# Jamy-L/Handheld-Multi-Frame-Super-Resolution

Measured on AMD Instinct MI355X. Metric: output Mpix/s for 12MP x 20-frame x2 SR burst; max-abs diff vs reference, higher is better.
Workload: dtype f32

## Files before the change

handheld-multi-frame-super-resolution_amd/csrc/hhsr_robustness.hip:

```cpp
#include "hhsr_common.h"

__device__ __forceinline__ double dodgson(double x) {
    const double a = fabs(x);
    if (a <= 0.5) return -2.0 * a * a + 1.0;
    if (a <= 1.5) return a * a - 5.0 / 2.0 * a + 1.5;
    return 0.0;
}

template <int NC>
__device__ __forceinline__ bool dodgson_sample(const float* __restrict__ LR, int lh, int lw, int y, int x, double fx,
                                               double fy, float out[NC]) {
    const double ly = ((double)y + fy + 0.5) / 2.0 - 0.5;
    const double lx = ((double)x + fx + 0.5) / 2.0 - 0.5;
    if (!(ly >= 0.0 && ly < (double)lh && lx >= 0.0 && lx < (double)lw)) return false;
    const int cy = (int)rint(ly), cx = (int)rint(lx);
    const size_t plane = (size_t)lh * lw;
    float b[NC];
#pragma unroll
    for (int c = 0; c < NC; ++c) b[c] = 0.f;
    double wacc = 0.0;
#pragma unroll
    for (int i = -1; i <= 1; ++i) {
        const int y_ = clampi(cy + i, 0, lh - 1);
        const double wy = dodgson((double)y_ - ly);
// ... 268 lines not shown
    w[1] = inner;
    w[2] = c + 1 <= len - 1 ? op : inner;
}

__global__ void __launch_bounds__(256) k_rob_frame_tile(const float* __restrict__ cm, int lh, int lw,
                                                         const float* __restrict__ rmean,
                                                         const float* __restrict__ ssq,
                                                         const uint32_t* __restrict__ cidx,
                                                         const float2* __restrict__ flow, int nx, int ts,
                                                         const float* __restrict__ S,
                                                         const double* __restrict__ difc, double t,
                                                         float* __restrict__ R, int H, int W) {
    __shared__ float s_g[2][2][3][RF_WN][RF_WN + 2];
    const int lx_ = threadIdx.x & (RF_BX - 1), ly_ = threadIdx.x >> 5;
    const int grp = lx_ >> 4;
    const int bx = blockIdx.x * RF_BX + grp * RF_T, by = blockIdx.y * RF_BY;
    const int x = blockIdx.x * RF_BX + lx_;
    const int tix = min(bx, W - 1) / ts;
    RobAxis ay[2], ax[2];
    int wy0[2], wx0[2];
    float Sv[2];
#pragma unroll
    for (int v = 0; v < 2; ++v) {
        const int tiy = min(by + RF_T * v, H - 1) / ts;
        const float2 f = flow[(size_t)tiy * nx + tix];
        Sv[v] = S[(size_t)tiy * nx + tix];
        ay[v] = rob_axis(f.y);
        ax[v] = rob_axis(f.x);
        float r_;
        rob_centre(ay[v], by + RF_T * v, lh, wy0[v], r_);
        rob_centre(ax[v], bx, lw, wx0[v], r_);
        wy0[v] = clampi(wy0[v], -4, lh + 4) - 1;
        wx0[v] = clampi(wx0[v], -4, lw + 4) - 1;
    }
    const size_t gplane = (size_t)lh * lw;
    const int tg = (lx_ & (RF_T - 1)) + RF_T * ly_;
    constexpr int WSZ = 3 * RF_WN * RF_WN, NST = (WSZ + 127) / 128;
    float st[2][NST];
#pragma unroll
    for (int v = 0; v < 2; ++v)
#pragma unroll
        for (int u = 0; u < NST; ++u) {
            const int p = tg + 128 * u;
            if (p < WSZ) {
                const int c = p / (RF_WN * RF_WN), q = p - c * (RF_WN * RF_WN);
                const int i = q / RF_WN, j = q - i * RF_WN;
                const int gy = clampi(wy0[v] + i, 0, lh - 1), gx = clampi(wx0[v] + j, 0, lw - 1);
                st[v][u] = cm[c * gplane + (size_t)gy * lw + gx];
            }
        }
    const size_t plane = (size_t)H * W;
    bool live[RF_NK];
    size_t o[RF_NK];
    float rb[RF_NK][3], s_sq[RF_NK];
    uint32_t ci[RF_NK];
#pragma unroll
    for (int k = 0; k < RF_NK; ++k) {
        const int y = by + ly_ + 8 * k;
        live[k] = x < W && y < H;
        o[k] = live[k] ? (size_t)y * W + x : 0;
#pragma unroll
        for (int c = 0; c < 3; ++c) rb[k][c] = rmean[c * plane + o[k]];
        s_sq[k] = ssq[o[k]];
        ci[k] = cidx[o[k]];
    }
#pragma unroll
    for (int v = 0; v < 2; ++v)
#pragma unroll
        for (int u = 0; u < NST; ++u) {
            const int p = tg + 128 * u;
            if (p < WSZ) {
                const int c = p / (RF_WN * RF_WN), q = p - c * (RF_WN * RF_WN);
                const int i = q / RF_WN, j = q - i * RF_WN;
                s_g[grp][v][c][i][j] = st[v][u];
            }
        }
    __syncthreads();
#pragma unroll
    for (int k = 0; k < RF_NK; ++k) {
        if (!live[k]) continue;
        const int v = k >> 1, y = by + ly_ + 8 * k;
        float d_t[3];
#pragma unroll
        for (int c = 0; c < 3; ++c) d_t[c] = (float)difc[(ci[k] >> (10 * c)) & 1023u];
        int cy, cx;
        float ry, rx;
        const bool iny = rob_centre(ay[v], y, lh, cy, ry), inx = rob_centre(ax[v], x, lw, cx, rx);
        float cmu[3] = {INFINITY, INFINITY, INFINITY};
        if (iny && inx) {
            float wxv[3], wyv[3], b0 = 0.f, b1 = 0.f, b2 = 0.f, wacc = 0.f;
            dodgson3(rx, cx, lw, wxv);
            dodgson3(ry, cy, lh, wyv);
            const int wi0 = cy - 1 - wy0[v], wj0 = cx - 1 - wx0[v];
#pragma unroll
            for (int i = 0; i < 3; ++i) {
#pragma unroll
                for (int j = 0; j < 3; ++j) {
                    const float w = wyv[i] * wxv[j];
                    b0 = fmaf(s_g[grp][v][0][wi0 + i][wj0 + j], w, b0);
                    b1 = fmaf(s_g[grp][v][1][wi0 + i][wj0 + j], w, b1);
                    b2 = fmaf(s_g[grp][v][2][wi0 + i][wj0 + j], w, b2);
                    wacc += w;
                }
            }
            const float iw = __builtin_amdgcn_rcpf(wacc);
            cmu[0] = b0 * iw;
            cmu[1] = b1 * iw;
            cmu[2] = b2 * iw;
        }
        float d_sq = 0.f;
#pragma unroll
        for (int c = 0; c < 3; ++c) {
            const float dp = fabsf(rb[k][c] - cmu[c]);
            const float dp2 = dp * dp;
            const float shrink = dp2 * __builtin_amdgcn_rcpf(dp2 + d_t[c] * d_t[c]);
            d_sq += dp2 * shrink * shrink;
        }
        const float e = __builtin_amdgcn_exp2f((-d_sq * __builtin_amdgcn_rcpf(s_sq[k])) * 1.44269504088896341f);
        double r = (double)(Sv[v] * e) - t;
        r = r > 0.0 ? r : 0.0;
        r = r < 1.0 ? r : 1.0;
        R[o[k]] = (float)r;
    }
}

__device__ __forceinline__ void rob_row4(const float (*win)[RF_WN][RF_WN + 2], const RobAxis& ay, const RobAxis& ax,
                                         int wy0, int wx0, int y, int x0, int lh, int lw, const float rbk[4][3],
                                         const float d_t2[4][3], const float iss[4], float Sv, float tf, float out[4]) {
    int cy;
    float ry, wyv[3];
    const bool iny = rob_centre(ay, y, lh, cy, ry);
    dodgson3(ry, cy, lh, wyv);
    const int wi0 = cy - 1 - wy0;
    float cmu[4][3];
#pragma unroll
    for (int ph = 0; ph < 2; ++ph) {
        int cx;
        float rx;
        const bool inx = rob_centre(ax, x0 + ph, lw, cx, rx);
#pragma unroll
        for (int c = 0; c < 3; ++c) cmu[ph][c] = cmu[ph + 2][c] = INFINITY;
        if (iny && inx && cx >= 1 && cx + 2 <= lw - 1) {
            float wxv[3], w[3][3], wacc = 0.f;
            dodgson3(rx, cx, lw, wxv);
#pragma unroll
            for (int i = 0; i < 3; ++i)
#pragma unroll
                for (int j = 0; j < 3; ++j) {
                    w[i][j] = wyv[i] * wxv[j];
                    wacc += w[i][j];
                }
            const float iw = __builtin_amdgcn_rcpf(wacc);
            const int wj0 = cx - 1 - wx0;
#pragma unroll
            for (int c = 0; c < 3; ++c) {
                float g4[3][4];
#pragma unroll
                for (int i = 0; i < 3; ++i)
#pragma unroll
                    for (int j = 0; j < 4; ++j) g4[i][j] = win[c][wi0 + i][wj0 + j];
#pragma unroll
                for (int q = 0; q < 2; ++q) {
                    float b = 0.f;
#pragma unroll
                    for (int i = 0; i < 3; ++i)
#pragma unroll
                        for (int j = 0; j < 3; ++j) b = fmaf(g4[i][j + q], w[i][j], b);
                    cmu[ph + 2 * q][c] = b * iw;
                }
            }
        } else {
            int cx2;
            float rx2;
            const bool inx2 = rob_centre(ax, x0 + ph + 2, lw, cx2, rx2);
#pragma unroll
            for (int q = 0; q < 2; ++q) {
                const int cxq = q ? cx2 : cx;
                const float rxq = q ? rx2 : rx;
                if (iny && (q ? inx2 : inx)) {
                    float wxv[3], b0 = 0.f, b1 = 0.f, b2 = 0.f, wacc = 0.f;
                    dodgson3(rxq, cxq, lw, wxv);
                    const int wj0 = cxq - 1 - wx0;
#pragma unroll
                    for (int i = 0; i < 3; ++i) {
#pragma unroll
                        for (int j = 0; j < 3; ++j) {
                            const float w = wyv[i] * wxv[j];
                            b0 = fmaf(win[0][wi0 + i][wj0 + j], w, b0);
                            b1 = fmaf(win[1][wi0 + i][wj0 + j], w, b1);
                            b2 = fmaf(win[2][wi0 + i][wj0 + j], w, b2);
                            wacc += w;
                        }
                    }
                    const float iw = __builtin_amdgcn_rcpf(wacc);
                    cmu[ph + 2 * q][0] = b0 * iw;
                    cmu[ph + 2 * q][1] = b1 * iw;
                    cmu[ph + 2 * q][2] = b2 * iw;
                }
            }
        }
    }
#pragma unroll
    for (int k = 0; k < 4; ++k) {
        float d_sq = 0.f;
#pragma unroll
        for (int c = 0; c < 3; ++c) {
            const float dp = fabsf(rbk[k][c] - cmu[k][c]);
            const float dp2 = dp * dp;
            const float shrink = dp2 * __builtin_amdgcn_rcpf(dp2 + d_t2[k][c]);
            d_sq += dp2 * shrink * shrink;
        }
        const float e = __builtin_amdgcn_exp2f((-d_sq * iss[k]) * 1.44269504088896341f);
        out[k] = __builtin_amdgcn_fmed3f(Sv * e - tf, 0.f, 1.f);
    }
}

__global__ void __launch_bounds__(256) k_rob_frame_row4(const float* __restrict__ cm, int lh, int lw,
                                                         const float* __restrict__ rmean,
                                                         const float* __restrict__ ssq,
                                                         const uint32_t* __restrict__ cidx,
                                                         const float2* __restrict__ flow, int nx, int ts,
                                                         const float* __restrict__ S,
                                                         const double* __restrict__ difc, double t,
                                                         float* __restrict__ R, int H, int W) {
    __shared__ float s_g[2][2][3][RF_WN][RF_WN + 2];
    const int lx4 = threadIdx.x & 7, ly_ = threadIdx.x >> 3;
    const int grp = lx4 >> 2, v = ly_ >> 4;
    const int bid = xcd_remap(blockIdx.y * gridDim.x + blockIdx.x, gridDim.x * gridDim.y);
    const int bxi = bid % gridDim.x, byi = bid / gridDim.x;
    const int sx0 = bxi * RF_BX + grp * RF_T, sy0 = byi * RF_BY + v * RF_T;
    const int x0 = bxi * RF_BX + 4 * lx4, y = byi * RF_BY + ly_;
    const int tix = min(sx0, W - 1) / ts, tiy = min(sy0, H - 1) / ts;
    const float2 f = flow[(size_t)tiy * nx + tix];
    const float Sv = S[(size_t)tiy * nx + tix];
    const RobAxis ay = rob_axis(f.y), ax = rob_axis(f.x);
    int wy0, wx0;
    {
        float r_;
        rob_centre(ay, sy0, lh, wy0, r_);
        rob_centre(ax, sx0, lw, wx0, r_);
        wy0 = clampi(wy0, -4, lh + 4) - 1;
        wx0 = clampi(wx0, -4, lw + 4) - 1;
    }
    const size_t gplane = (size_t)lh * lw;
    const int tg = (ly_ & (RF_T - 1)) * 4 + (lx4 & 3);
    constexpr int WSZ = 3 * RF_WN * RF_WN, NST = (WSZ + 63) / 64;
    float st[NST];
#pragma unroll
    for (int u = 0; u < NST; ++u) {
        const int p = tg + 64 * u;
        if (p < WSZ) {
            const int c = p / (RF_WN * RF_WN), q = p - c * (RF_WN * RF_WN);
            const int i = q / RF_WN, j = q - i * RF_WN;
            const int gy = clampi(wy0 + i, 0, lh - 1), gx = clampi(wx0 + j, 0, lw - 1);
            st[u] = cm[c * gplane + (size_t)gy * lw + gx];
        }
    }
    const size_t plane = (size_t)H * W;
    const bool live = x0 < W && y < H;
    const size_t o = live ? (size_t)y * W + x0 : 0;
    float4 rb4[3];
#pragma unroll
    for (int c = 0; c < 3; ++c) rb4[c] = *reinterpret_cast<const float4*>(rmean + c * plane + o);
    const float4 ss4 = *reinterpret_cast<const float4*>(ssq + o);
    const uint4 ci4 = *reinterpret_cast<const uint4*>(cidx + o);
#pragma unroll
    for (int u = 0; u < NST; ++u) {
        const int p = tg + 64 * u;
        if (p < WSZ) {
            const int c = p / (RF_WN * RF_WN), q = p - c * (RF_WN * RF_WN);
            const int i = q / RF_WN, j = q - i * RF_WN;
            s_g[grp][v][c][i][j] = st[u];
        }
    }
    __syncthreads();
    if (!live) return;
    const float rbk[4][3] = {{rb4[0].x, rb4[1].x, rb4[2].x}, {rb4[0].y, rb4[1].y, rb4[2].y},
                             {rb4[0].z, rb4[1].z, rb4[2].z}, {rb4[0].w, rb4[1].w, rb4[2].w}};
    const float ssk[4] = {ss4.x, ss4.y, ss4.z, ss4.w};
    const uint32_t cik[4] = {ci4.x, ci4.y, ci4.z, ci4.w};
    float d_t2[4][3], iss[4], out[4];
#pragma unroll
    for (int k = 0; k < 4; ++k) {
#pragma unroll
        for (int c = 0; c < 3; ++c) {
            const float d = (float)difc[(cik[k] >> (10 * c)) & 1023u];
            d_t2[k][c] = d * d;
        }
        iss[k] = __builtin_amdgcn_rcpf(ssk[k]);
    }
    rob_row4(s_g[grp][v], ay, ax, wy0, wx0, y, x0, lh, lw, rbk, d_t2, iss, Sv, (float)t, out);
    *reinterpret_cast<float4*>(R + o) = make_float4(out[0], out[1], out[2], out[3]);
}

constexpr int ROB_GROUP = 4;
struct RobGroup {
    const float* cm[ROB_GROUP];
    const float2* flow[ROB_GROUP];
    const float* S[ROB_GROUP];
    float* R[ROB_GROUP];
    int n;
};

__global__ void __launch_bounds__(256) k_rob_frames_row4(RobGroup gq, int lh, int lw, const float* __restrict__ rmean,
                                                          const float* __restrict__ ssq,
                                                          const uint32_t* __restrict__ cidx, int ny, int nx, int ts,
                                                          const double* __restrict__ difc, double t, int H, int W,
                                                          double Mt2, float s1, float s2, int rows_lo, int rows_hi) {
    __shared__ float s_g[2][2][3][RF_WN][RF_WN + 2];
    __shared__ float4 s_tab[ROB_GROUP][2][2][2];
    const int lx4 = threadIdx.x & 7, ly_ = threadIdx.x >> 3;
    const int grp = lx4 >> 2, v = ly_ >> 4;
    const int bid = xcd_remap(blockIdx.y * gridDim.x + blockIdx.x, gridDim.x * gridDim.y);
    const int bxi = bid % gridDim.x, byi = bid / gridDim.x;
    const int x0 = bxi * RF_BX + 4 * lx4, y = byi * RF_BY + ly_;
    const size_t gplane = (size_t)lh * lw, plane = (size_t)H * W;
    const int tg = (ly_ & (RF_T - 1)) * 4 + (lx4 & 3);
    constexpr int WSZ = 3 * RF_WN * RF_WN, NST = (WSZ + 63) / 64;
    const bool live = x0 < W && y < H;
    const size_t o = live ? (size_t)y * W + x0 : 0;
    float4 rb4[3];
#pragma unroll
    for (int c = 0; c < 3; ++c) rb4[c] = *reinterpret_cast<const float4*>(rmean + c * plane + o);
    const float4 ss4 = *reinterpret_cast<const float4*>(ssq + o);
    const uint4 ci4 = *reinterpret_cast<const uint4*>(cidx + o);
    const float rbk[4][3] = {{rb4[0].x, rb4[1].x, rb4[2].x}, {rb4[0].y, rb4[1].y, rb4[2].y},
                             {rb4[0].z, rb4[1].z, rb4[2].z}, {rb4[0].w, rb4[1].w, rb4[2].w}};
    const float ssk[4] = {ss4.x, ss4.y, ss4.z, ss4.w};
    const uint32_t cik[4] = {ci4.x, ci4.y, ci4.z, ci4.w};
    float d_t2[4][3], iss[4];
#pragma unroll
    for (int k = 0; k < 4; ++k) {
#pragma unroll
        for (int c = 0; c < 3; ++c) {
            const float d = (float)difc[(cik[k] >> (10 * c)) & 1023u];
            d_t2[k][c] = d * d;
        }
        iss[k] = __builtin_amdgcn_rcpf(ssk[k]);
    }
    if (threadIdx.x < gq.n * 4) {
        const int fr = threadIdx.x >> 2, vv = (threadIdx.x >> 1) & 1, gg = threadIdx.x & 1;
        const int tsx0 = bxi * RF_BX + gg * RF_T, tsy0 = byi * RF_BY + vv * RF_T;
        const size_t tl = (size_t)(min(tsy0, H - 1) / ts) * nx + min(tsx0, W - 1) / ts;
        const float2 f = gq.flow[fr][tl];
        const RobAxis ay = rob_axis(f.y), ax = rob_axis(f.x);
        int wy0, wx0;
        float r_;
        rob_centre(ay, tsy0, lh, wy0, r_);
        rob_centre(ax, tsx0, lw, wx0, r_);
        wy0 = clampi(wy0, -4, lh + 4) - 1;
        wx0 = clampi(wx0, -4, lw + 4) - 1;
        const int flags = (ay.lt ? 1 : 0) | (ay.eq ? 2 : 0) | (ay.ok ? 4 : 0) | (ax.lt ? 8 : 0) | (ax.eq ? 16 : 0) | (ax.ok ? 32 : 0);
        s_tab[fr][vv][gg][0] = make_float4(__int_as_float(ay.fi), ay.h, __int_as_float(wy0), __int_as_float(flags));
        float Sv;
        if (gq.S[fr]) {
            Sv = gq.S[fr][tl];
        } else {
            const int tiy = (int)(tl / nx), tix = (int)(tl - (size_t)tiy * nx);
            float mnx = INFINITY, mny = INFINITY, mxx = -INFINITY, mxy = -INFINITY;
            for (int i = -1; i <= 1; ++i)
                for (int j = -1; j <= 1; ++j) {
                    const int yy = tiy + i, xx = tix + j;
                    if (yy >= -rows_lo && yy < ny + rows_hi && xx >= 0 && xx < nx) {
                        const float2 q = gq.flow[fr][(ptrdiff_t)yy * nx + xx];
                        mxx = fmaxf(mxx, q.x); mxy = fmaxf(mxy, q.y);
                        mnx = fminf(mnx, q.x); mny = fminf(mny, q.y);
                    }
                }
            const float d0 = mxx - mnx, d1 = mxy - mny;
            const float m = d0 * d0 + d1 * d1;
            Sv = ((double)m > Mt2) ? s1 : s2;
        }
        s_tab[fr][vv][gg][1] = make_float4(__int_as_float(ax.fi), ax.h, __int_as_float(wx0), Sv);
    }
    __syncthreads();
    float st[NST];
    int fci[NST];
    unsigned fco[NST];
#pragma unroll
    for (int u = 0; u < NST; ++u) {
        const int p = tg + 64 * u;
        const int c = p / (RF_WN * RF_WN), q = p - c * (RF_WN * RF_WN);
        const int i = q / RF_WN, j = q - i * RF_WN;
        fci[u] = (i << 8) | j;
        fco[u] = (unsigned)c * (unsigned)gplane;
    }
    auto fetch = [&](int fr) {
        const float* __restrict__ cm = gq.cm[fr];
        const int wy0 = __float_as_int(s_tab[fr][v][grp][0].z), wx0 = __float_as_int(s_tab[fr][v][grp][1].z);
#pragma unroll
        for (int u = 0; u < NST; ++u) {
            const int p = tg + 64 * u;
            if (p < WSZ) {
                const int gy = clampi(wy0 + (fci[u] >> 8), 0, lh - 1), gx = clampi(wx0 + (fci[u] & 255), 0, lw - 1);
                const unsigned off = (fco[u] + (unsigned)(__mul24(gy, lw) + gx)) * 4u;
                st[u] = *reinterpret_cast<const float*>(reinterpret_cast<const char*>(cm) + off);
            }
        }
    };
    if (gq.n > 0) fetch(0);
    for (int fr = 0; fr < gq.n; ++fr) {
        const float4 t0 = s_tab[fr][v][grp][0], t1 = s_tab[fr][v][grp][1];
        const int flags = __float_as_int(t0.w);
        RobAxis ay, ax;
        ay.fi = __float_as_int(t0.x); ay.h = t0.y; ay.lt = flags & 1; ay.eq = flags & 2; ay.ok = flags & 4;
        ax.fi = __float_as_int(t1.x); ax.h = t1.y; ax.lt = flags & 8; ax.eq = flags & 16; ax.ok = flags & 32;
        const int wy0 = __float_as_int(t0.z), wx0 = __float_as_int(t1.z);
        const float Sv = t1.w;
        if (fr) __syncthreads();
#pragma unroll
        for (int u = 0; u < NST; ++u) {
            const int p = tg + 64 * u;
            if (p < WSZ) {
                const int c = p / (RF_WN * RF_WN), q = p - c * (RF_WN * RF_WN);
                const int i = q / RF_WN, j = q - i * RF_WN;
                s_g[grp][v][c][i][j] = st[u];
            }
        }
        __syncthreads();
        if (fr + 1 < gq.n) fetch(fr + 1);
        if (!live) continue;
        float out[4];
        rob_row4(s_g[grp][v], ay, ax, wy0, wx0, y, x0, lh, lw, rbk, d_t2, iss, Sv, (float)t, out);
        *reinterpret_cast<float4*>(gq.R[fr] + o) = make_float4(out[0], out[1], out[2], out[3]);
    }
}

extern "C" int hhsr_rob_frame(const float* comp_means, int lh, int lw, const float* ref_means,
                              const float* ref_sigma_sq, const uint32_t* ref_curve_index, const float* flow, int ny,
                              int nx, int ts, const float* S, const double* diff_curve, int ncurve, double t, float* R,
                              void* stream) {
    HHSR_ARG(comp_means && ref_means && ref_sigma_sq && flow && S && diff_curve && R);
    HHSR_ARG(lh > 0 && lw > 0 && ts > 0 && ncurve > 0);
    const int H = 2 * lh, W = 2 * lw;
    HHSR_ARG(ny * ts >= H && nx * ts >= W);
    const bool vec4 = W % 4 == 0 && (((uintptr_t)ref_means | (uintptr_t)ref_sigma_sq | (uintptr_t)ref_curve_index |
                                      (uintptr_t)R) & 15) == 0;
    if (ts % RF_T == 0 && ref_curve_index && ncurve <= 1024 && vec4)
        hipLaunchKernelGGL(k_rob_frame_row4, dim3(hhsr_cdiv(W, RF_BX), hhsr_cdiv(H, RF_BY)), dim3(256), 0,
                           (hipStream_t)stream, comp_means, lh, lw, ref_means, ref_sigma_sq, ref_curve_index,
                           reinterpret_cast<const float2*>(flow), nx, ts, S, diff_curve, t, R, H, W);
    else if (ts % RF_T == 0 && ref_curve_index && ncurve <= 1024)
        hipLaunchKernelGGL(k_rob_frame_tile, dim3(hhsr_cdiv(W, RF_BX), hhsr_cdiv(H, RF_BY)), dim3(256), 0,
                           (hipStream_t)stream, comp_means, lh, lw, ref_means, ref_sigma_sq, ref_curve_index,
                           reinterpret_cast<const float2*>(flow), nx, ts, S, diff_curve, t, R, H, W);
    else
        hipLaunchKernelGGL(k_rob_frame, dim3(hhsr_cdiv(W, 64), hhsr_cdiv(H, 4)), dim3(256), 0, (hipStream_t)stream,
                           comp_means, lh, lw, ref_means, ref_sigma_sq, reinterpret_cast<const float2*>(flow), nx, ts,
                           S, diff_curve, ncurve, t, R, H, W);
    HHSR_LAUNCHED();
}

extern "C" int hhsr_rob_frames(const float* const* comp_means, int n_frames, int lh, int lw, const float* ref_means,
                               const float* ref_sigma_sq, const uint32_t* ref_curve_index, const float* const* flows,
                               int ny, int nx, int ts, const float* const* S, double Mt, float s1, float s2,
                               const double* diff_curve, int ncurve, double t, float* const* R, int flow_rows_before,
                               int flow_rows_after, void* stream) {
    HHSR_ARG(comp_means && flows && R && n_frames >= 0 && flow_rows_before >= 0 && flow_rows_after >= 0);
    for (int n = 0; n < n_frames; ++n) HHSR_ARG(comp_means[n] && flows[n] && (!S || S[n]) && R[n]);
    HHSR_ARG(ref_means && ref_sigma_sq && diff_curve && lh > 0 && lw > 0 && ts > 0 && ncurve > 0);
    const int H = 2 * lh, W = 2 * lw;
    HHSR_ARG(ny * ts >= H && nx * ts >= W);
    bool vec4 = W % 4 == 0 && (((uintptr_t)ref_means | (uintptr_t)ref_sigma_sq | (uintptr_t)ref_curve_index) & 15) == 0;
    for (int n = 0; n < n_frames; ++n) vec4 = vec4 && ((uintptr_t)R[n] & 15) == 0;
    if (!(ts % RF_T == 0 && ref_curve_index && ncurve <= 1024 && vec4)) {
        if (!S) {
            hhsr_set_error("hhsr_rob_frames: S = NULL (weights evaluated inside the kernel) needs the grouped kernel: "
                           "ts %% 16 == 0, W %% 4 == 0, packed curve indices, 16-byte aligned planes");
            return -3;
        }
        for (int n = 0; n < n_frames; ++n) {
            const int rc = hhsr_rob_frame(comp_means[n], lh, lw, ref_means, ref_sigma_sq, ref_curve_index, flows[n], ny, nx,
                                          ts, S[n], diff_curve, ncurve, t, R[n], stream);
            if (rc) return rc;
        }
        return 0;
    }
    for (int n0 = 0; n0 < n_frames; n0 += ROB_GROUP) {
        RobGroup g;
        g.n = n_frames - n0 < ROB_GROUP ? n_frames - n0 : ROB_GROUP;
        for (int k = 0; k < ROB_GROUP; ++k) {
            const int n = n0 + (k < g.n ? k : 0);
            g.cm[k] = comp_means[n];
            g.flow[k] = reinterpret_cast<const float2*>(flows[n]);
            g.S[k] = S ? S[n] : nullptr;
            g.R[k] = R[n];
        }
        hipLaunchKernelGGL(k_rob_frames_row4, dim3(hhsr_cdiv(W, RF_BX), hhsr_cdiv(H, RF_BY)), dim3(256), 0,
                           (hipStream_t)stream, g, lh, lw, ref_means, ref_sigma_sq, ref_curve_index, ny, nx, ts, diff_curve, t,
                           H, W, Mt * Mt, s1, s2, flow_rows_before, flow_rows_after);
    }
    HHSR_LAUNCHED();
}

constexpr int LM_TX = 64, LM_TY = 16;

__global__ void __launch_bounds__(256) k_local_min5(const float* __restrict__ R, int H, int W,
                                                     float* __restrict__ r, float* __restrict__ acc) {
    __shared__ float s[LM_TY + 4][LM_TX + 4 + 1];
    __shared__ float s_row[LM_TY + 4][LM_TX + 1];
    const int x0 = blockIdx.x * LM_TX, y0 = blockIdx.y * LM_TY;
    for (int p = threadIdx.x; p < (LM_TY + 4) * (LM_TX + 4); p += 256) {
        const int i = p / (LM_TX + 4), j = p - i * (LM_TX + 4);
        s[i][j] = R[(size_t)clampi(y0 + i - 2, 0, H - 1) * W + clampi(x0 + j - 2, 0, W - 1)];
    }
    __syncthreads();
    for (int p = threadIdx.x; p < (LM_TY + 4) * LM_TX; p += 256) {
        const int i = p / LM_TX, j = p - i * LM_TX;
        float m = s[i][j];
#pragma unroll
        for (int k = 1; k < 5; ++k) m = fminf(m, s[i][j + k]);
        s_row[i][j] = m;
    }
    __syncthreads();
    for (int p = threadIdx.x; p < LM_TY * LM_TX; p += 256) {
        const int i = p / LM_TX, j = p - i * LM_TX;
        const int y = y0 + i, x = x0 + j;
        if (y < H && x < W) {
            float m = s_row[i][j];
#pragma unroll
            for (int k = 1; k < 5; ++k) m = fminf(m, s_row[i + k][j]);
            r[(size_t)y * W + x] = m;
            if (acc) acc[(size_t)y * W + x] += m;
        }
    }
}

extern "C" int hhsr_local_min5(const float* R, int H, int W, float* r, float* acc_r, void* stream) {
    HHSR_ARG(R && r && H > 0 && W > 0 && R != r);
    hipLaunchKernelGGL(k_local_min5, dim3(hhsr_cdiv(W, LM_TX), hhsr_cdiv(H, LM_TY)), dim3(256), 0,
                       (hipStream_t)stream, R, H, W, r, acc_r);
    HHSR_LAUNCHED();
}

struct RobSumFrames {
    const float* r[HHSR_MAX_FRAMES];
    int n;
};

__global__ void __launch_bounds__(256) k_rob_sum(RobSumFrames fr, size_t count, int load, double mfc, float m32, float below,
                                                  float above, double* __restrict__ sum64, float* __restrict__ mask32,
                                                  float* __restrict__ dec32) {
    const size_t i = (size_t)blockIdx.x * 256 + threadIdx.x;
    if (i >= count) return;
    double s = load ? sum64[i] : 0.0;
    for (int n = 0; n < fr.n; ++n) s += (double)fr.r[n][i];
    if (sum64) sum64[i] = s;
    float a = (float)s;
    if (mask32) mask32[i] = a;
    if (dec32) {
        if (s < mfc && a >= m32) a = below;
        if (s > mfc && a <= m32) a = above;
        dec32[i] = a;
    }
}

__global__ void __launch_bounds__(256) k_rob_sum_min5(RobSumFrames fr, int H, int W, int load, double mfc, float m32,
                                                       float below, float above, double* __restrict__ sum64,
                                                       float* __restrict__ mask32, float* __restrict__ dec32) {
    __shared__ float s[LM_TY + 4][LM_TX + 4 + 1];
    __shared__ float s_row[LM_TY + 4][LM_TX + 1];
    constexpr int NIN = ((LM_TY + 4) * (LM_TX + 4) + 255) / 256, NROW = (LM_TY + 4) * LM_TX / 256, NOUT = LM_TY * LM_TX / 256;
    const int x0 = blockIdx.x * LM_TX, y0 = blockIdx.y * LM_TY, tid = threadIdx.x;
    unsigned off[NIN];
#pragma unroll
    for (int u = 0; u < NIN; ++u) {
        const int p = tid + 256 * u, i = p / (LM_TX + 4), j = p - i * (LM_TX + 4);
        off[u] = (unsigned)(clampi(y0 + i - 2, 0, H - 1) * W + clampi(x0 + j - 2, 0, W - 1));
    }
    double acc[NOUT];
#pragma unroll
    for (int u = 0; u < NOUT; ++u) {
        const int p = tid + 256 * u, i = p / LM_TX, j = p - i * LM_TX;
        const bool live = y0 + i < H && x0 + j < W;
        acc[u] = (load && live) ? sum64[(size_t)(y0 + i) * W + x0 + j] : 0.0;
    }
    float pre[NIN];
    auto fetch = [&](int n) {
#pragma unroll
        for (int u = 0; u < NIN; ++u)
            if (tid + 256 * u < (LM_TY + 4) * (LM_TX + 4)) pre[u] = fr.r[n][off[u]];
    };
    if (fr.n > 0) fetch(0);
    for (int n = 0; n < fr.n; ++n) {
#pragma unroll
        for (int u = 0; u < NIN; ++u) {
            const int p = tid + 256 * u, i = p / (LM_TX + 4), j = p - i * (LM_TX + 4);
            if (p < (LM_TY + 4) * (LM_TX + 4)) s[i][j] = pre[u];
        }
        __syncthreads();
        if (n + 1 < fr.n) fetch(n + 1);
#pragma unroll
        for (int u = 0; u < NROW; ++u) {
            const int p = tid + 256 * u, i = p / LM_TX, j = p - i * LM_TX;
            float m = s[i][j];
#pragma unroll
            for (int k = 1; k < 5; ++k) m = fminf(m, s[i][j + k]);
            s_row[i][j] = m;
        }
        __syncthreads();
#pragma unroll
        for (int u = 0; u < NOUT; ++u) {
            const int p = tid + 256 * u, i = p / LM_TX, j = p - i * LM_TX;
            float m = s_row[i][j];
#pragma unroll
            for (int k = 1; k < 5; ++k) m = fminf(m, s_row[i + k][j]);
            acc[u] += (double)m;
        }
    }
#pragma unroll
    for (int u = 0; u < NOUT; ++u) {
        const int p = tid + 256 * u, i = p / LM_TX, j = p - i * LM_TX;
        if (y0 + i >= H || x0 + j >= W) continue;
        const size_t o = (size_t)(y0 + i) * W + x0 + j;
        const double sv = acc[u];
        if (sum64) sum64[o] = sv;
        float a = (float)sv;
        if (mask32) mask32[o] = a;
        if (dec32) {
            if (sv < mfc && a >= m32) a = below;
            if (sv > mfc && a <= m32) a = above;
            dec32[o] = a;
        }
    }
}
static_assert((LM_TY + 4) * LM_TX % 256 == 0 && LM_TY * LM_TX % 256 == 0, "k_rob_sum_min5: whole passes per thread");

extern "C" int hhsr_rob_sum(const float* const* rs, int n_frames, int H, int W, int flags, double max_frame_count,
                            double* sum64, float* mask32, float* decisions32, void* stream) {
    const int load = flags & HHSR_ROB_SUM_LOAD;
    HHSR_ARG(n_frames >= 0 && n_frames <= HHSR_MAX_FRAMES && H > 0 && W > 0);
    HHSR_ARG(!(flags & ~(HHSR_ROB_SUM_LOAD | HHSR_ROB_SUM_MIN5)));
    HHSR_ARG(n_frames == 0 || rs != nullptr);
    HHSR_ARG(!load || sum64 != nullptr);
    HHSR_ARG(sum64 || mask32 || decisions32);
    RobSumFrames fr;
    fr.n = n_frames;
    for (int k = 0; k < HHSR_MAX_FRAMES; ++k) {
        fr.r[k] = k < n_frames ? rs[k] : nullptr;
        HHSR_ARG(k >= n_frames || rs[k] != nullptr);
    }
    const float m32 = (float)max_frame_count;
    const float below = (double)m32 < max_frame_count ? m32 : nextafterf(m32, -INFINITY);
    const float above = (double)m32 > max_frame_count ? m32 : nextafterf(m32, INFINITY);
    const size_t count = (size_t)H * W;
    if ((flags & HHSR_ROB_SUM_MIN5) && n_frames > 0) {
        HHSR_ARG(count < ((size_t)1 << 32));
        hipLaunchKernelGGL(k_rob_sum_min5, dim3(hhsr_cdiv(W, LM_TX), hhsr_cdiv(H, LM_TY)), dim3(256), 0, (hipStream_t)stream,
                           fr, H, W, load, max_frame_count, m32, below, above, sum64, mask32, decisions32);
        HHSR_LAUNCHED();
    }
    hipLaunchKernelGGL(k_rob_sum, dim3((unsigned)((count + 255) / 256)), dim3(256), 0, (hipStream_t)stream, fr, count, load,
                       max_frame_count, m32, below, above, sum64, mask32, decisions32);
    HHSR_LAUNCHED();
}

__global__ void __launch_bounds__(256) k_mono_rob_upscale(const float* __restrict__ LR, int H, int W,
                                                           const float2* __restrict__ flow, int nx, int ts,
                                                           float* __restrict__ HR) {
    const int x = blockIdx.x * 64 + (threadIdx.x & 63), y = blockIdx.y * 4 + (threadIdx.x >> 6);
    if (x >= W || y >= H) return;
    double fx = 0.0, fy = 0.0;
    if (flow) {
        const float2 f = flow[(size_t)(y / ts) * nx + x / ts];
        fx = (double)f.x;
        fy = (double)f.y;
    }
    float v[1];
    if (!dodgson_sample<1>(LR, H, W, y, x, fx, fy, v)) v[0] = INFINITY;
    HR[(size_t)y * W + x] = v[0];
}

extern "C" int hhsr_mono_rob_upscale(const float* stats, int H, int W, const float* flow, int ny, int nx, int ts,
                                     float* out, void* stream) {
    HHSR_ARG(stats && out && H > 0 && W > 0);
    if (flow) HHSR_ARG(ts > 0 && (int64_t)ny * ts >= H && (int64_t)nx * ts >= W);
    hipLaunchKernelGGL(k_mono_rob_upscale, dim3(hhsr_cdiv(W, 64), hhsr_cdiv(H, 4)), dim3(256), 0, (hipStream_t)stream,
                       stats, H, W, reinterpret_cast<const float2*>(flow), nx, ts > 0 ? ts : 1, out);
    HHSR_LAUNCHED();
}

__global__ void __launch_bounds__(256) k_mono_rob_sigma(const float* __restrict__ rmean, const float* __restrict__ rvar,
                                                         const double* __restrict__ stdc, int ncurve,
                                                         float* __restrict__ ssq, size_t n) {
    const size_t o = (size_t)blockIdx.x * blockDim.x + threadIdx.x;
    if (o >= n) return;
    int id = 0;
    const double bb = 1000.0 * (double)rmean[o];
    if (isfinite(bb)) id = clampi((int)rint(bb), 0, ncurve - 1);
    const double s_t = stdc[id], st2 = s_t * s_t, sp = (double)rvar[o];
    ssq[o] = (float)(0.0 + ((st2 > sp) ? st2 : sp));
}

extern "C" int hhsr_mono_rob_sigma(const float* ref_means, const float* ref_vars, int H, int W,
                                   const double* std_curve, int ncurve, float* sigma_sq, void* stream) {
    HHSR_ARG(ref_means && ref_vars && std_curve && sigma_sq && H > 0 && W > 0 && ncurve > 0);
    const size_t n = (size_t)H * W;
    hipLaunchKernelGGL(k_mono_rob_sigma, dim3((unsigned)((n + 255) / 256)), dim3(256), 0, (hipStream_t)stream,
                       ref_means, ref_vars, std_curve, ncurve, sigma_sq, n);
    HHSR_LAUNCHED();
}

__global__ void __launch_bounds__(256) k_mono_rob_frame(const float* __restrict__ cm, const float* __restrict__ rmean,
                                                         const float* __restrict__ ssq,
                                                         const float2* __restrict__ flow, int nx, int ts,
                                                         const float* __restrict__ S, const double* __restrict__ difc,
                                                         int ncurve, double t, float* __restrict__ R, int H, int W) {
    const int x = blockIdx.x * 64 + (threadIdx.x & 63), y = blockIdx.y * 4 + (threadIdx.x >> 6);
    if (x >= W || y >= H) return;
    const int tix = x / ts, tiy = y / ts;
    const float2 f = flow[(size_t)tiy * nx + tix];
    float cmu[1];
    if (!dodgson_sample<1>(cm, H, W, y, x, (double)f.x, (double)f.y, cmu)) cmu[0] = INFINITY;
    const size_t o = (size_t)y * W + x;
    const float b = rmean[o];
    const float dp = fabsf(b - cmu[0]);
    int id = 0;
    const double bb = 1000.0 * (double)b;
    if (isfinite(bb)) id = clampi((int)rint(bb), 0, ncurve - 1);
    const double d_t = difc[id];
    const float dp2f = dp * dp;
    const double dp2 = (double)dp2f;
    const double shrink = dp2 / (dp2 + d_t * d_t);
    const double d_sq = 0.0 + dp2 * shrink * shrink;
    const float dsf = (float)d_sq, ssf = ssq[o];
    const float e = expf(-dsf / ssf);
    double v = (double)(S[(size_t)tiy * nx + tix] * e) - t;
    v = v > 0.0 ? v : 0.0;
    v = v < 1.0 ? v : 1.0;
    R[o] = (float)v;
}

__global__ void __launch_bounds__(256) k_mono_rob_frame4(const float* __restrict__ cm, const float* __restrict__ rmean,
                                                          const float* __restrict__ ssq,
                                                          const float2* __restrict__ flow, int nx, int ts,
                                                          const float* __restrict__ S, const double* __restrict__ difc,
                                                          int ncurve, float tf, float* __restrict__ R, int H, int W) {
    const int x0 = (blockIdx.x * 16 + (threadIdx.x & 15)) * 4, y = blockIdx.y * 16 + (threadIdx.x >> 4);
    if (x0 >= W || y >= H) return;
    const int tix = x0 / ts, tiy = y / ts;
    const float2 f = flow[(size_t)tiy * nx + tix];
    const float Sv = S[(size_t)tiy * nx + tix];
    const RobAxis ay = rob_axis(f.y), ax = rob_axis(f.x);
    const size_t o = (size_t)y * W + x0;
    const float4 rb4 = *reinterpret_cast<const float4*>(rmean + o);
    const float4 ss4 = *reinterpret_cast<const float4*>(ssq + o);
    const float rbk[4] = {rb4.x, rb4.y, rb4.z, rb4.w}, ssk[4] = {ss4.x, ss4.y, ss4.z, ss4.w};
    int cy, cx[4];
    float ry, rx[4], wyv[3];
    bool inx[4];
    const bool iny = rob_centre(ay, y, H, cy, ry);
    dodgson3(ry, cy, H, wyv);
#pragma unroll
    for (int k = 0; k < 4; ++k) inx[k] = rob_centre(ax, x0 + k, W, cx[k], rx[k]);
    const float* row[3];
#pragma unroll
    for (int i = 0; i < 3; ++i) row[i] = cm + (size_t)clampi(cy - 1 + i, 0, H - 1) * W;
    float cmu[4] = {INFINITY, INFINITY, INFINITY, INFINITY};
    if (iny && inx[0] && inx[1] && !ax.eq && cx[0] >= 1 && cx[1] + 2 <= W - 1) {
        const int c0 = cx[0] - 1;
        const bool d = cx[1] != cx[0];
        float g[3][5];
#pragma unroll
// ... 80 lines not shown
```

Measured before the change: 6229.

## Precompute per-tile Dodgson weight tables and use a shifted LDS window for interior tiles

In the grouped robustness kernel, each tile's 3x3 Dodgson interpolation weights are now computed once per frame, tile and phase by sixteen setup threads and stored in shared memory. Interior tiles (valid flow, not on the boundary) take a fast path that reads those weights and gathers the window from LDS with paired float2 loads. To keep those loads aligned, the window is written twice, the second copy shifted by one element. Non-interior tiles keep the original per-pixel weight evaluation, using the old layout encoded in the upper bits of a packed destination offset. This removes repeated per-pixel weight evaluation, at the cost of more LDS use, more stores, and a new argument limit on plane size.

```diff
diff --git a/handheld-multi-frame-super-resolution_amd/csrc/hhsr_robustness.hip b/handheld-multi-frame-super-resolution_amd/csrc/hhsr_robustness.hip
--- a/handheld-multi-frame-super-resolution_amd/csrc/hhsr_robustness.hip
+++ b/handheld-multi-frame-super-resolution_amd/csrc/hhsr_robustness.hip
@@ -594,13 +594,64 @@
     int n;
 };
 
+constexpr int RT_PITCH = 12, RT_CH = RF_WN * RT_PITCH;
+constexpr int RT_COPY = 448, RT_SUB = 928;
+typedef float rob_f2 __attribute__((ext_vector_type(2)));
+typedef __attribute__((address_space(3))) rob_f2 rob_lds_f2;
+static_assert(RT_COPY % 64 == 0 && RT_SUB % 64 == 32 && 3 * RT_CH <= RT_COPY && RT_COPY + 3 * RT_CH <= RT_SUB &&
+              3 * RF_WN * (RF_WN + 2) <= RT_SUB, "window layout");
+
+__device__ __forceinline__ void rob_row4_tab(const float* __restrict__ win, const float tw[20], int row, const int xo[2],
+                                             const float rbk[4][3], const float d_t2[4][3], const float iss[4], float Sv,
+                                             float tf, float out[4]) {
+    float cmu[4][3];
+#pragma unroll
+    for (int ph = 0; ph < 2; ++ph) {
+        const float* w = tw + 10 * ph;
+        const float iw = w[9];
+#pragma unroll
+        for (int c = 0; c < 3; ++c) {
+            float g4[3][4];
+#pragma unroll
+            for (int i = 0; i < 3; ++i) {
+                const volatile rob_lds_f2* g = (const volatile rob_lds_f2*)(win + c * RT_CH + i * RT_PITCH + row + xo[ph]);
+                const rob_f2 lo = g[0], hi = g[1];
+                g4[i][0] = lo.x; g4[i][1] = lo.y; g4[i][2] = hi.x; g4[i][3] = hi.y;
+            }
+#pragma unroll
+            for (int q = 0; q < 2; ++q) {
+                float b = 0.f;
+#pragma unroll
+                for (int i = 0; i < 3; ++i)
+#pragma unroll
+                    for (int j = 0; j < 3; ++j) b = fmaf(g4[i][j + q], w[3 * i + j], b);
+                cmu[ph + 2 * q][c] = b * iw;
+            }
+        }
+    }
+#pragma unroll
+    for (int k = 0; k < 4; ++k) {
+        float d_sq = 0.f;
+#pragma unroll
+        for (int c = 0; c < 3; ++c) {
+            const float dp = fabsf(rbk[k][c] - cmu[k][c]);
+            const float dp2 = dp * dp;
+            const float shrink = dp2 * __builtin_amdgcn_rcpf(dp2 + d_t2[k][c]);
+            d_sq += dp2 * shrink * shrink;
+        }
+        const float e = __builtin_amdgcn_exp2f((-d_sq * iss[k]) * 1.44269504088896341f);
+        out[k] = __builtin_amdgcn_fmed3f(Sv * e - tf, 0.f, 1.f);
+    }
+}
+
 __global__ void __launch_bounds__(256) k_rob_frames_row4(RobGroup gq, int lh, int lw, const float* __restrict__ rmean,
                                                           const float* __restrict__ ssq,
                                                           const uint32_t* __restrict__ cidx, int ny, int nx, int ts,
                                                           const double* __restrict__ difc, double t, int H, int W,
                                                           double Mt2, float s1, float s2, int rows_lo, int rows_hi) {
-    __shared__ float s_g[2][2][3][RF_WN][RF_WN + 2];
+    __shared__ __attribute__((aligned(16))) float s_w[4 * RT_SUB];
     __shared__ float4 s_tab[ROB_GROUP][2][2][2];
+    __shared__ float4 s_wt[ROB_GROUP][2][5][2][2];
     const int lx4 = threadIdx.x & 7, ly_ = threadIdx.x >> 3;
     const int grp = lx4 >> 2, v = ly_ >> 4;
     const int bid = xcd_remap(blockIdx.y * gridDim.x + blockIdx.x, gridDim.x * gridDim.y);
@@ -630,8 +681,9 @@
         }
         iss[k] = __builtin_amdgcn_rcpf(ssk[k]);
     }
-    if (threadIdx.x < gq.n * 4) {
-        const int fr = threadIdx.x >> 2, vv = (threadIdx.x >> 1) & 1, gg = threadIdx.x & 1;
+    if (threadIdx.x < gq.n * 16) {
+        const int fr = threadIdx.x >> 4, vv = (threadIdx.x >> 3) & 1, gg = (threadIdx.x >> 2) & 1;
+        const int yph = (threadIdx.x >> 1) & 1, xpx = threadIdx.x & 1;
         const int tsx0 = bxi * RF_BX + gg * RF_T, tsy0 = byi * RF_BY + vv * RF_T;
         const size_t tl = (size_t)(min(tsy0, H - 1) / ts) * nx + min(tsx0, W - 1) / ts;
         const float2 f = gq.flow[fr][tl];
@@ -640,35 +692,61 @@
         float r_;
         rob_centre(ay, tsy0, lh, wy0, r_);
         rob_centre(ax, tsx0, lw, wx0, r_);
+        const bool interior = ay.ok && ax.ok && !ay.eq && !ax.eq && wy0 >= 1 && wy0 + 9 <= lh - 1 && wx0 >= 1 &&
+                              wx0 + 9 <= lw - 1;
         wy0 = clampi(wy0, -4, lh + 4) - 1;
         wx0 = clampi(wx0, -4, lw + 4) - 1;
-        const int flags = (ay.lt ? 1 : 0) | (ay.eq ? 2 : 0) | (ay.ok ? 4 : 0) | (ax.lt ? 8 : 0) | (ax.eq ? 16 : 0) | (ax.ok ? 32 : 0);
-        s_tab[fr][vv][gg][0] = make_float4(__int_as_float(ay.fi), ay.h, __int_as_float(wy0), __int_as_float(flags));
-        float Sv;
-        if (gq.S[fr]) {
-            Sv = gq.S[fr][tl];
-        } else {
-            const int tiy = (int)(tl / nx), tix = (int)(tl - (size_t)tiy * nx);
-            float mnx = INFINITY, mny = INFINITY, mxx = -INFINITY, mxy = -INFINITY;
-            for (int i = -1; i <= 1; ++i)
-                for (int j = -1; j <= 1; ++j) {
-                    const int yy = tiy + i, xx = tix + j;
-                    if (yy >= -rows_lo && yy < ny + rows_hi && xx >= 0 && xx < nx) {
-                        const float2 q = gq.flow[fr][(ptrdiff_t)yy * nx + xx];
-                        mxx = fmaxf(mxx, q.x); mxy = fmaxf(mxy, q.y);
-                        mnx = fminf(mnx, q.x); mny = fminf(mny, q.y);
+        {
+            int c_;
+            float ry, rx, wyv[3], wxv[3], wacc = 0.f;
+            rob_centre(ay, yph - ay.fi, lh, c_, ry);
+            rob_centre(ax, xpx, lw, c_, rx);
+            dodgson3(ry, 1, 3, wyv);
+            dodgson3(rx, 1, 3, wxv);
+            float* wt = reinterpret_cast<float*>(&s_wt[fr][vv][0][gg][yph]);
+#pragma unroll
+            for (int i = 0; i < 3; ++i)
+#pragma unroll
+                for (int j = 0; j < 3; ++j) {
+                    const float w = wyv[i] * wxv[j];
+                    wacc += w;
+                    const int e = 10 * xpx + 3 * i + j;
+                    wt[(e >> 2) * 16 + (e & 3)] = w;
+                }
+            const int e = 10 * xpx + 9;
+            wt[(e >> 2) * 16 + (e & 3)] = __builtin_amdgcn_rcpf(wacc);
+        }
+        if ((threadIdx.x & 3) == 0) {
+            const int flags = (ay.lt ? 1 : 0) | (ay.eq ? 2 : 0) | (ay.ok ? 4 : 0) | (ax.lt ? 8 : 0) | (ax.eq ? 16 : 0) |
+                              (ax.ok ? 32 : 0) | (interior ? 64 : 0);
+            s_tab[fr][vv][gg][0] = make_float4(__int_as_float(ay.fi), ay.h, __int_as_float(wy0), __int_as_float(flags));
+            float Sv;
+            if (gq.S[fr]) {
+                Sv = gq.S[fr][tl];
+            } else {
+                const int tiy = (int)(tl / nx), tix = (int)(tl - (size_t)tiy * nx);
+                float mnx = INFINITY, mny = INFINITY, mxx = -INFINITY, mxy = -INFINITY;
+                for (int i = -1; i <= 1; ++i)
+                    for (int j = -1; j <= 1; ++j) {
+                        const int yy = tiy + i, xx = tix + j;
+                        if (yy >= -rows_lo && yy < ny + rows_hi && xx >= 0 && xx < nx) {
+                            const float2 q = gq.flow[fr][(ptrdiff_t)yy * nx + xx];
+                            mxx = fmaxf(mxx, q.x); mxy = fmaxf(mxy, q.y);
+                            mnx = fminf(mnx, q.x); mny = fminf(mny, q.y);
+                        }
                     }
-                }
-            const float d0 = mxx - mnx, d1 = mxy - mny;
-            const float m = d0 * d0 + d1 * d1;
-            Sv = ((double)m > Mt2) ? s1 : s2;
-        }
-        s_tab[fr][vv][gg][1] = make_float4(__int_as_float(ax.fi), ax.h, __int_as_float(wx0), Sv);
+                const float d0 = mxx - mnx, d1 = mxy - mny;
+                const float m = d0 * d0 + d1 * d1;
+                Sv = ((double)m > Mt2) ? s1 : s2;
+            }
+            s_tab[fr][vv][gg][1] = make_float4(__int_as_float(ax.fi), ax.h, __int_as_float(wx0), Sv);
+        }
     }
     __syncthreads();
     float st[NST];
     int fci[NST];
     unsigned fco[NST];
+    unsigned dst[NST];
 #pragma unroll
     for (int u = 0; u < NST; ++u) {
         const int p = tg + 64 * u;
@@ -676,7 +754,10 @@
         const int i = q / RF_WN, j = q - i * RF_WN;
         fci[u] = (i << 8) | j;
         fco[u] = (unsigned)c * (unsigned)gplane;
-    }
+        const int sub = (v * 2 + grp) * RT_SUB;
+        dst[u] = (unsigned)(sub + c * RT_CH + i * RT_PITCH + j) * 4u | (unsigned)(sub + (c * RF_WN + i) * (RF_WN + 2) + j) << 18;
+    }
+    const float* const sw = s_w + (v * 2 + grp) * RT_SUB;
     auto fetch = [&](int fr) {
         const float* __restrict__ cm = gq.cm[fr];
         const int wy0 = __float_as_int(s_tab[fr][v][grp][0].z), wx0 = __float_as_int(s_tab[fr][v][grp][1].z);
@@ -694,26 +775,44 @@
     for (int fr = 0; fr < gq.n; ++fr) {
         const float4 t0 = s_tab[fr][v][grp][0], t1 = s_tab[fr][v][grp][1];
         const int flags = __float_as_int(t0.w);
-        RobAxis ay, ax;
-        ay.fi = __float_as_int(t0.x); ay.h = t0.y; ay.lt = flags & 1; ay.eq = flags & 2; ay.ok = flags & 4;
-        ax.fi = __float_as_int(t1.x); ax.h = t1.y; ax.lt = flags & 8; ax.eq = flags & 16; ax.ok = flags & 32;
+        const bool tabbed = flags & 64;
         const int wy0 = __float_as_int(t0.z), wx0 = __float_as_int(t1.z);
         const float Sv = t1.w;
         if (fr) __syncthreads();
-#pragma unroll
-        for (int u = 0; u < NST; ++u) {
-            const int p = tg + 64 * u;
-            if (p < WSZ) {
-                const int c = p / (RF_WN * RF_WN), q = p - c * (RF_WN * RF_WN);
-                const int i = q / RF_WN, j = q - i * RF_WN;
-                s_g[grp][v][c][i][j] = st[u];
-            }
-        }
+        const int half = tabbed ? 0 : 16;
+#pragma unroll
+        for (int u = 0; u < NST; ++u)
+            if (tg + 64 * u < WSZ) {
+                float* d = reinterpret_cast<float*>(reinterpret_cast<char*>(s_w) + ((dst[u] >> half) & 0xffffu));
+                d[0] = st[u];
+                if (tabbed) d[RT_COPY - 1] = st[u];
+            }
         __syncthreads();
         if (fr + 1 < gq.n) fetch(fr + 1);
         if (!live) continue;
         float out[4];
-        rob_row4(s_g[grp][v], ay, ax, wy0, wx0, y, x0, lh, lw, rbk, d_t2, iss, Sv, (float)t, out);
+        if (tabbed) {
+            const int ny_ = y + __float_as_int(t0.x), fix = __float_as_int(t1.x);
+            const int yph = ny_ & 1, cy = (ny_ >> 1) + ((flags & 1) ? 0 : yph);
+            const float4* wt = &s_wt[fr][v][0][grp][yph];
+            const float4 q0 = wt[0], q1 = wt[4], q2 = wt[8], q3 = wt[12], q4 = wt[16];
+            const float tw[20] = {q0.x, q0.y, q0.z, q0.w, q1.x, q1.y, q1.z, q1.w, q2.x, q2.y,
+                                  q2.z, q2.w, q3.x, q3.y, q3.z, q3.w, q4.x, q4.y, q4.z, q4.w};
+            int xo[2];
+#pragma unroll
+            for (int ph = 0; ph < 2; ++ph) {
+                const int nx_ = x0 + ph + fix, cx = (nx_ >> 1) + ((flags & 8) ? 0 : (nx_ & 1));
+                const int wj0 = cx - 1 - wx0;
+                xo[ph] = (wj0 & ~1) + (wj0 & 1) * RT_COPY;
+            }
+            rob_row4_tab(sw, tw, (cy - 1 - wy0) * RT_PITCH, xo, rbk, d_t2, iss, Sv, (float)t, out);
+        } else {
+            RobAxis ay, ax;
+            ay.fi = __float_as_int(t0.x); ay.h = t0.y; ay.lt = flags & 1; ay.eq = flags & 2; ay.ok = flags & 4;
+            ax.fi = __float_as_int(t1.x); ax.h = t1.y; ax.lt = flags & 8; ax.eq = flags & 16; ax.ok = flags & 32;
+            rob_row4(reinterpret_cast<const float (*)[RF_WN][RF_WN + 2]>(sw), ay, ax, wy0, wx0, y, x0, lh, lw, rbk, d_t2,
+                     iss, Sv, (float)t, out);
+        }
         *reinterpret_cast<float4*>(gq.R[fr] + o) = make_float4(out[0], out[1], out[2], out[3]);
     }
 }
@@ -751,6 +850,7 @@
     HHSR_ARG(comp_means && flows && R && n_frames >= 0 && flow_rows_before >= 0 && flow_rows_after >= 0);
     for (int n = 0; n < n_frames; ++n) HHSR_ARG(comp_means[n] && flows[n] && (!S || S[n]) && R[n]);
     HHSR_ARG(ref_means && ref_sigma_sq && diff_curve && lh > 0 && lw > 0 && ts > 0 && ncurve > 0);
+    HHSR_ARG(lh < (1 << 23) && lw < (1 << 23) && 3ull * (unsigned long long)lh * (unsigned long long)lw * 4ull < (1ull << 32));
     const int H = 2 * lh, W = 2 * lw;
     HHSR_ARG(ny * ts >= H && nx * ts >= W);
     bool vec4 = W % 4 == 0 && (((uintptr_t)ref_means | (uintptr_t)ref_sigma_sq | (uintptr_t)ref_curve_index) & 15) == 0;
```

Result: no change. 6271, median of 6 (+0.7%).
